# pallgeuer/novic

Hardware: NVIDIA B200
Metric: labels/sec (greedy, batch 4096) (higher is better)
Workload: dtype bf16

## Files before the change

novic_b200/csrc/abi.cu:

```cuda
#include <cstdarg>
#include <cstdio>
#include <cstring>
#include <map>
#include <mutex>
#include <string>
#include <tuple>
#include <vector>

#include "../../include/novic_b200.h"
#include "train.cuh"
#include "optim.cuh"
#include "vit.cuh"
#include "blockrows.cuh"

using namespace novic;

namespace {

thread_local std::string g_err;
int64_t g_launches = 0;

int fail(const char* fmt, ...) {
  char buf[1024];
  va_list ap;
// ... 107 lines not shown

int make_tmap_3d(CUtensorMap* map, const void* base, const cuuint64_t (&dims)[3], const cuuint64_t (&strides)[2], const cuuint32_t (&box)[3]) {
  if (load_driver_entry()) return 1;
  if ((reinterpret_cast<uintptr_t>(base) & 15) != 0 || strides[0] % 16 != 0 || strides[1] % 16 != 0) return fail("TMA operand base / strides must be 16-byte aligned");
  if (box[0] * 2 != 128) return fail("128-byte swizzle needs a 64-element inner box");
  cuuint32_t estr[3] = {1, 1, 1};
  CUresult r = g_encode(map, CU_TENSOR_MAP_DATA_TYPE_BFLOAT16, 3, const_cast<void*>(base), dims, strides, box, estr, CU_TENSOR_MAP_INTERLEAVE_NONE,
                        CU_TENSOR_MAP_SWIZZLE_128B, CU_TENSOR_MAP_L2_PROMOTION_L2_256B, CU_TENSOR_MAP_FLOAT_OOB_FILL_NONE);
  if (r != CUDA_SUCCESS) return fail("cuTensorMapEncodeTiled (3-D) failed with CUresult %d", (int)r);
  return 0;
}

constexpr int kStagesQKV = 5, kStagesGelu = 5, kStagesRow = 4, kStagesLogits = 5;
bool g_fuse_block = true;
int g_block_rows64_min = 148 * 32 + 1;
int g_attn_split_max = 0;
int g_qkv_ws_div = 24;
int g_qkv_ws_stages = 3;
int g_vit_direct = 1;
bool g_attn_prefix = true;
bool g_attn_split = true;
bool g_fuse_attn = false;
bool g_ffn1_ksplit = true;
int g_block64_pad = 16384;
int g_block_rows = 0;
constexpr int kBlock64MaxRows = 1536;
int g_qkv_ws = 1;
bool g_wgrad_mn = true;
int g_qkv_per_tile = 0;
int g_qkv_mc = 0;
int g_qkv_bn = 128;
bool g_fuse_qkv = false;
bool g_attn_tf = true;
int g_attn_hint = 1;
int g_row_stages = 4;
bool g_split_ffn = true;
bool g_early_b = true;
bool g_wide_gemm = true;
constexpr int kWideKbs = 2, kWideStages = 3;
int g_num_sms = 148;
int g_logits_ew = 16;
int g_logits_bn = 256;
int g_grid_div = 1;
constexpr int kLogitBN = kTileN;

bool g_use_pdl = true;
int g_cur_class = 9;
unsigned g_skip_classes = 0;
template <class... KArgs, class... Args>
cudaError_t launch_k(void (*kernel)(KArgs...), dim3 grid, dim3 block, size_t smem, cudaStream_t s, Args&&... args) {
  if ((g_skip_classes >> g_cur_class) & 1u) return cudaSuccess;
  cudaLaunchConfig_t cfg{};
  cfg.gridDim = grid; cfg.blockDim = block; cfg.dynamicSmemBytes = smem; cfg.stream = s;
  cudaLaunchAttribute attr[1];
  attr[0].id = cudaLaunchAttributeProgrammaticStreamSerialization;
  attr[0].val.programmaticStreamSerializationAllowed = 1;
  cfg.attrs = attr; cfg.numAttrs = g_use_pdl ? 1 : 0;
  return cudaLaunchKernelEx(&cfg, kernel, static_cast<KArgs>(args)...);
}

template <class Epi, int STAGES, int KBS = 1, int BN = kTileN, int EW = kEpiWarps>
int set_gemm_attr() {
  static_assert(gemm_persistent_smem_bytes(STAGES, KBS, BN, EW) <= 227 * 1024, "GEMM pipeline does not fit in shared memory");
  CUDA_TRY(cudaFuncSetAttribute(gemm_kernel<Epi, STAGES, KBS, BN, EW>, cudaFuncAttributeMaxDynamicSharedMemorySize, gemm_persistent_smem_bytes(STAGES, KBS, BN, EW)));
  return 0;
}

// ... 283 lines not shown
};

struct Workspace {
  int64_t B = 0, nseq = 0, rows = 0, logit_rows = 0;
  int H = 1, rps = 0, ntiles = 0, hcap = 0, chains = 1;
  float* ein; __nv_bfloat16* ebf; float* x; __nv_bfloat16 *xn, *xfin, *q, *ao, *hb; __nv_bfloat16* kv;
  LogitPartial* part; float* topv; int* topi;
  long long* g_tok; unsigned char *g_pad, *g_done; float *g_score, *g_nll, *g_len, *g_score_out; int* flags;
  long long* b_tok[2]; unsigned char *b_pad[2], *b_anc[2], *b_fin[2]; float *b_score[2], *b_len[2], *b_norm;
  unsigned char *keypad, *effpad, *correct; long long* tgt_masked; float *nll_rows, *loss;
  uint32_t* allow = nullptr; int allow_words = 0; int* allow_edge0 = nullptr; int* g_node = nullptr; int* b_node[2] = {nullptr, nullptr};
  size_t bytes = 0;
};

struct GraphKey {
  int mode; int64_t B; int H; float tau, alpha; void* ws;
  const void* guide = nullptr; int guide_flags = 0;
  const void* bias = nullptr;
  const void* guide_tok = nullptr; const void* guide_node = nullptr; int num_nodes = 0, num_edges = 0;
  bool operator<(const GraphKey& o) const {
    return std::tie(mode, B, H, tau, alpha, ws, guide, guide_flags, bias, guide_tok, guide_node, num_nodes, num_edges) <
           std::tie(o.mode, o.B, o.H, o.tau, o.alpha, o.ws, o.guide, o.guide_flags, o.bias, o.guide_tok, o.guide_node, o.num_nodes, o.num_edges);
  }
};

struct NovicHandle {
  NovicCfg cfg;
  int device = 0;
  bool weights_set = false;
  bool use_graphs = true;
  bool attn_v1 = false;
  int attn_early = 1;
  int attn_cfg = 0;
  bool attn_stream = true;
  bool fuse_ffn = true;
  bool split_sms = true;
  int num_sms = 148;
  int max_chains = 1;
  cudaStream_t chain_streams[8] = {};
  cudaEvent_t fork_ev = nullptr, join_ev[8] = {};
  int attn_smem_budget = 200 * 1024;
  DropCfg drop_in{nullptr, 0u, 1.f}, drop_layer{nullptr, 0u, 1.f};
  uint32_t* d_drop_seed = nullptr;
  uint32_t drop_seed = 0;
  const void* wbuf_seen = nullptr;
  bool train_graphs = true;
  std::map<std::vector<uint64_t>, std::pair<cudaGraphExec_t, cudaGraphExec_t>> train_graph_cache;
  std::map<std::vector<uint64_t>, int64_t> train_graph_nodes;
  WeightPtrs w;
  cudaStream_t capture_stream = nullptr;
  std::map<GraphKey, cudaGraphExec_t> graphs;
  std::map<GraphKey, int64_t> graph_nodes;
  int* h_flags = nullptr;
  int G() const { return cfg.token_length - 1; }
  int S() const { return cfg.prefix_len + cfg.token_length - 1; }
};

namespace {

int plan_workspace(const NovicHandle* h, int64_t B, int H, int rps, char* base, Workspace* ws) {
  const NovicCfg& c = h->cfg;
  const int P = c.prefix_len, G = h->G(), S = h->S();
  Workspace w;
  w.B = B; w.H = H; w.rps = rps;
  w.nseq = B * H;
  const bool tf = rps > 0;
// ... 36 lines not shown
    w.g_score = reinterpret_cast<float*>(P_(4 * B));
    w.g_nll = reinterpret_cast<float*>(P_(4 * B));
    w.g_len = reinterpret_cast<float*>(P_(4 * B));
    w.g_score_out = reinterpret_cast<float*>(P_(4 * B));
  } else if (!tf) {
    for (int i = 0; i < 2; ++i) {
      w.b_tok[i] = reinterpret_cast<long long*>(P_(8 * w.nseq * G));
      w.b_pad[i] = reinterpret_cast<unsigned char*>(P_(w.nseq * G));
      w.b_anc[i] = reinterpret_cast<unsigned char*>(P_(w.nseq * G));
      w.b_fin[i] = reinterpret_cast<unsigned char*>(P_(w.nseq));
      w.b_score[i] = reinterpret_cast<float*>(P_(4 * w.nseq));
      w.b_len[i] = reinterpret_cast<float*>(P_(4 * w.nseq));
    }
    w.b_norm = reinterpret_cast<float*>(P_(4 * w.nseq));
  } else {
    w.keypad = reinterpret_cast<unsigned char*>(P_(w.nseq * S));
    w.effpad = reinterpret_cast<unsigned char*>(P_(w.logit_rows));
    w.correct = reinterpret_cast<unsigned char*>(P_(w.logit_rows));
    w.tgt_masked = reinterpret_cast<long long*>(P_(8 * w.logit_rows));
    w.nll_rows = reinterpret_cast<float*>(P_(4 * w.logit_rows));
    w.loss = reinterpret_cast<float*>(P_(4 * 2));
  }
  w.bytes = b.off;
  *ws = w;
  return 0;
}

struct PassCfg {
  int M;
  int nseq, nq, q0, slot_mul, beams;
  const unsigned char* keypad; int keypad_ld;
  const unsigned char* anc; int anc_ld;
  int remap_in, remap_skip, remap_out;
};

AttnParams attention_params(NovicHandle* h, const Workspace& ws, const PassCfg& pc, int l) {
  const NovicCfg& c = h->cfg;
  const int S = h->S();
  const size_t kv_layer = static_cast<size_t>(ws.nseq) * S * kE;
  __nv_bfloat16* kc = ws.kv + (static_cast<size_t>(l) * 2 + 0) * kv_layer;
  __nv_bfloat16* vc = ws.kv + (static_cast<size_t>(l) * 2 + 1) * kv_layer;
  AttnParams pa{};
  pa.q = ws.q; pa.kcache = kc; pa.vcache = vc; pa.out = ws.ao; pa.keypad = pc.keypad; pa.anc = pc.anc;
  pa.nseq = pc.nseq; pa.nq = pc.nq; pa.q0 = pc.q0; pa.smax = S; pa.P = c.prefix_len; pa.beams = pc.beams;
  pa.prefix_bidir = c.strictly_causal ? 0 : 1; pa.keypad_ld = pc.keypad_ld; pa.anc_ld = pc.anc_ld;
  pa.slot_mul = pc.slot_mul;
  pa.early_loads = h->attn_early;
  pa.scale_log2e = 1.4426950408889634f / sqrtf(static_cast<float>(kHeadDim));
  pa.stream_hint = g_attn_hint;
  return pa;
}

int launch_attention(NovicHandle* h, const Workspace& ws, const PassCfg& pc, int l, cudaStream_t s) {
  const NovicCfg& c = h->cfg;
  const AttnParams pa = attention_params(h, ws, pc, l);
  KSpan t(kKAttn, s);
  const int nkeys_step = (pa.prefix_bidir && pc.q0 < pa.P) ? pa.P : pc.q0 + 1;
  if (h->attn_stream && g_attn_split && pc.nq == 1 && pc.keypad == nullptr && nkeys_step <= kSpMaxKeys &&
      pc.nseq <= (g_attn_split_max > 0 ? g_attn_split_max : 2 * kSpSeqs * std::max(1, h->num_sms / g_grid_div))) {
    CUDA_TRY(launch_k(attention_split_kernel, dim3(static_cast<unsigned>(ceil_div(pc.nseq, kSpSeqs))), dim3(kSpWarps * 32), kSpSmemBytes, s, pa));
  } else if (h->attn_stream && pc.nq == 1 && pc.keypad == nullptr) {
    auto go = [&](auto kernel, int warps, int slots, int chunk) {
      const int grid = static_cast<int>(std::min<int64_t>(std::max(1, h->num_sms / g_grid_div), ceil_div(pc.nseq, warps)));
      return launch_k(kernel, dim3(grid), dim3(warps * 32), as_smem_bytes(warps, slots, chunk), s, pa);
    };
    switch (h->attn_cfg) {
      case 1: CUDA_TRY(go(attention_stream_kernel_t<12, 2, 8>, 12, 2, 8)); break;
      case 2: CUDA_TRY(go(attention_stream_kernel_t<16, 2, 6>, 16, 2, 6)); break;
      case 3: CUDA_TRY(go(attention_stream_kernel_t<8, 3, 8>, 8, 3, 8)); break;
      case 4: CUDA_TRY(go(attention_stream_kernel_t<24, 2, 4>, 24, 2, 4)); break;
      case 5: CUDA_TRY(go(attention_stream_kernel_t<14, 3, 4>, 14, 3, 4)); break;
      case 6: CUDA_TRY(go(attention_stream_kernel_t<14, 4, 4>, 14, 4, 4)); break;
      case 7: CUDA_TRY(go(attention_stream_kernel_t<28, 2, 4>, 28, 2, 4)); break;
      case 8: CUDA_TRY(go(attention_stream_kernel_t<16, 2, 4>, 16, 2, 4)); break;
      default: CUDA_TRY(go(attention_stream_kernel_t<16, 3, 4>, 16, 3, 4)); break;
    }
  } else if (g_attn_prefix && pc.q0 == 0 && pc.nq == c.prefix_len && pc.nq <= kApMaxP && pc.keypad == nullptr && pc.anc == nullptr) {
    const int grid = static_cast<int>(std::min<int64_t>(std::max(1, h->num_sms / g_grid_div), ceil_div(pc.nseq, kApWarps)));
    CUDA_TRY(launch_k(attention_prefix_kernel, dim3(grid), dim3(kApWarps * 32), kApSmemBytes, s, pa));
  } else if (g_attn_tf && pc.q0 == 0 && pc.nq > c.prefix_len && pc.nq <= kAttnBwdMaxS && pc.beams == 1 && pc.slot_mul == 1 && pc.anc == nullptr) {
    const unsigned grid = static_cast<unsigned>(ceil_div(static_cast<int64_t>(pc.nseq) * kHeads, kAttnTfWarps));
    attention_tf_kernel<false><<<grid, kAttnTfWarps * 32, kAttnTfSmemBytes, s>>>(pa);
// ... 5 lines not shown
    const int stage_bytes = nk_max * 2048;
    const int budget = h->attn_smem_budget;
    int nstages = std::max(2, std::min(kAttnMaxStages, (budget - 512) / stage_bytes));
    const int ncons = std::min(kAttnConsumers, nstages);
    nstages = nstages / ncons * ncons;
    const int smem = nstages * stage_bytes + 2 * kAttnMaxStages * 8;
    const int grid = static_cast<int>(std::min<int64_t>(std::max(1, h->num_sms / g_grid_div), ceil_div(pc.nseq, 2)));
    CUDA_TRY(launch_k(attention_bulk_kernel, dim3(grid), dim3(kAttnThreads), smem, s, pa, nstages, stage_bytes, ncons));
  }
  ++g_launches;
  return 0;
}

int run_layers(NovicHandle* h, const Workspace& ws, const PassCfg& pc, cudaStream_t s) {
  const NovicCfg& c = h->cfg;
  const int L = c.num_layers, S = h->S(), M = pc.M;
  CUtensorMap tm_xn, tm_ao, tm_hb;
  if (make_tmap(&tm_xn, ws.xn, M, kE, kBlockM)) return 1;
  if (make_tmap(&tm_ao, ws.ao, M, kE, kBlockM)) return 1;
  if (make_tmap(&tm_hb, ws.hb, M, c.ffn_dim, kBlockM)) return 1;
  CUtensorMap tm_xn3, tm_ao64;
  if (make_tmap3(&tm_xn3, ws.xn, M, kE, kBlockM, kWideKbs)) return 1;
  if (make_tmap3(&tm_ao64, ws.ao, M, kE, kHbRows, 2)) return 1;
  CUtensorMap tm_ao32;
  if (make_tmap3(&tm_ao32, ws.ao, M, kE, kBrRows, kE / kBlockK)) return 1;
  CUtensorMap tm_ao64r;
  if (make_tmap3(&tm_ao64r, ws.ao, M, kE, kB64Rows, kE / kBlockK)) return 1;
  const bool rows64 = g_block_rows64_min > 0 && M >= g_block_rows64_min;
  CUtensorMap tm_x_st;
  if (make_tmap_xblk(&tm_x_st, ws.x, static_cast<int64_t>(ceil_div(M, 32)) * 32)) return 1;
  const size_t kv_layer = static_cast<size_t>(ws.nseq) * S * kE;
  const bool block_fused = g_fuse_block && h->fuse_ffn && c.ffn_dim == kFfnDim;
  const bool qkv_tail = block_fused && g_fuse_qkv && g_wide_gemm;
  auto qkv_params = [&](int l) {
    __nv_bfloat16* kc = ws.kv + (static_cast<size_t>(l) * 2 + 0) * kv_layer;
    __nv_bfloat16* vc = ws.kv + (static_cast<size_t>(l) * 2 + 1) * kv_layer;
    return EpiQKV::Params{ws.q, kc, vc, pc.nq, pc.q0, pc.slot_mul, S, (g_attn_hint & 2) ? 1 : 0};
  };
  for (int l = 0; l < L; ++l) {
    if (l == 0 || !qkv_tail) {
      const EpiQKV::Params pq = qkv_params(l);
      if (g_wide_gemm) {
        KSpan t(kKQkv, s);
        if (g_qkv_ws && kE == kWsKb * kBlockK && ceil_div(M, kBlockM) * g_qkv_ws_div >= 2 * (g_num_sms / g_grid_div / (3 * kE / kTileN))) {
          if (g_qkv_ws == 2) {
            if (launch_gemm_ws2<EpiQKV>(s, tm_xn3, h->w.tm_in_proj3h[l], M, 3 * kE, pq, g_early_b)) return 1;
          } else if (g_qkv_ws_stages == 3) {
            if (launch_gemm_ws<EpiQKV, 3>(s, tm_xn3, h->w.tm_in_proj3[l], M, 3 * kE, pq, g_early_b, &tm_xn)) return 1;
          } else if (launch_gemm_ws<EpiQKV, 2>(s, tm_xn3, h->w.tm_in_proj3[l], M, 3 * kE, pq, g_early_b, &tm_xn)) return 1;
        } else if (g_qkv_bn == 512 && ceil_div(M, kBlockM) * (3 * kE / 256) >= g_num_sms) {
          if (launch_gemm2<EpiQKV, 3>(s, tm_xn3, h->w.tm_in_proj3[l], M, 3 * kE, kE, pq, g_early_b)) return 1;
        } else if (g_qkv_bn == 384 && ceil_div(M, 2 * kBlockM) * (3 * kE / 128) >= g_num_sms / 2) {
          if (launch_gemm2<EpiQKV, 4, 128>(s, tm_xn3, h->w.tm_in_proj3h[l], M, 3 * kE, kE, pq, g_early_b)) return 1;
        } else if (g_qkv_bn == 256 && ceil_div(M, kBlockM) * (3 * kE / 256) >= g_num_sms) {
          if (launch_gemm<EpiQKV, 2, kWideKbs, 256>(s, tm_xn3, h->w.tm_in_proj3w[l], M, 3 * kE, kE, pq, 1, g_early_b)) return 1;
        } else if (launch_gemm<EpiQKV, kWideStages, kWideKbs>(s, tm_xn3, h->w.tm_in_proj3[l], M, 3 * kE, kE, pq, 1, g_early_b)) return 1;
      } else {
        KSpan t(kKQkv, s);
        if (launch_gemm<EpiQKV, kStagesQKV>(s, tm_xn, h->w.tm_in_proj[l], M, 3 * kE, kE, pq, 1, g_early_b)) return 1;
      }
    }
    const bool attn_in_block = block_fused && !qkv_tail && (g_block_rows == 32 || g_block_rows == 0) && g_fuse_attn && h->attn_stream && pc.nq == 1 &&
                               pc.keypad == nullptr;
    if (!attn_in_block && launch_attention(h, ws, pc, l, s)) return 1;
    if (block_fused) {
      FusedBlockParams fb{};
      fb.x = ws.x; fb.gain_mid = h->w.norm2[l]; fb.eps = c.ln_eps;
      if (l + 1 < L) {
        fb.xn = ws.xn; fb.gain_out = h->w.norm1[l + 1];
        if (qkv_tail) { fb.qkv_tail = 1; fb.qkv = qkv_params(l + 1); }
      } else {
        fb.gain_out = h->w.final_norm;
        fb.xn = pc.remap_in > 0 ? ws.xfin : ws.xn;
        fb.remap_rows_in = pc.remap_in; fb.remap_skip = pc.remap_skip; fb.remap_rows_out = pc.remap_out;
      }
      KSpan t(kKFfn2, s);
      if ((g_block_rows == 32 || g_block_rows == 0) && !fb.qkv_tail) {
        const AttnParams pa = attention_params(h, ws, pc, l);
        if (launch_block_rows(s, tm_ao32, h->w.tm_out_proj4[l], h->w.tm_linear1_r3[l], h->w.tm_linear2_4[l], tm_x_st, M, fb, attn_in_block ? &pa : nullptr,
                              (rows64 && !attn_in_block) ? &tm_ao64r : nullptr)) return 1;
        continue;
      }
      if ((g_block_rows == 64 || (g_block_rows <= 0 && M <= kBlock64MaxRows)) && !fb.qkv_tail) {
        if (launch_outproj_ffn64(s, tm_ao64, h->w.tm_out_proj3[l], h->w.tm_linear1_q3[l], h->w.tm_linear2_3[l], M, fb)) return 1;
        continue;
      }
      if (g_ffn1_ksplit && !fb.qkv_tail) {
        if (launch_outproj_ffn_ks(s, tm_ao, h->w.tm_out_proj[l], h->w.tm_linear1[l], h->w.tm_linear2[l], M, fb)) return 1;
        continue;
      }
      if (launch_outproj_ffn(s, tm_ao, h->w.tm_out_proj[l], h->w.tm_linear1_q[l], h->w.tm_linear2[l], h->w.tm_in_proj3[l + 1 < L ? l + 1 : l], M, fb)) return 1;
      continue;
    }
    RowParams po{};
    po.x = ws.x; po.xn = ws.xn; po.gain = h->w.norm2[l]; po.pos = nullptr; po.eps = c.ln_eps;
    { KSpan t(kKOutProj, s); if (launch_rowln(s, tm_ao, h->w.tm_out_proj[l], M, kE, kE, po)) return 1; }
    RowParams pf{};
    pf.x = ws.x; pf.pos = nullptr; pf.eps = c.ln_eps;
    if (l + 1 < L) {
      pf.xn = ws.xn; pf.gain = h->w.norm1[l + 1];
    } else {
      pf.gain = h->w.final_norm;
      pf.xn = pc.remap_in > 0 ? ws.xfin : ws.xn;
      pf.remap_rows_in = pc.remap_in; pf.remap_skip = pc.remap_skip; pf.remap_rows_out = pc.remap_out;
    }
    if (h->fuse_ffn) {
      KSpan t(kKFfn2, s);
// ... 92 lines not shown
  ++g_launches;
  return 0;
}

int enqueue_greedy(NovicHandle* h, const Workspace& ws, float tau, float alpha, float* logits, const GuideCfg& guide, cudaStream_t s) {
  const NovicCfg& c = h->cfg;
  g_grid_div = h->split_sms ? ws.chains : 1;
  const int B = static_cast<int>(ws.B), P = c.prefix_len, G = h->G(), V = c.vocab_size;
  const float inv_tau = 1.0f / tau;
  CUDA_TRY(cudaMemsetAsync(ws.g_done, 0, B, s));
  CUDA_TRY(cudaMemsetAsync(ws.g_score, 0, 4 * B, s));
  CUDA_TRY(cudaMemsetAsync(ws.g_nll, 0, 4 * B, s));
  CUDA_TRY(cudaMemsetAsync(ws.g_len, 0, 4 * B, s));
  CUDA_TRY(cudaMemsetAsync(ws.flags, 1, sizeof(int) * (G + 2), s));
  if (guide.on) CUDA_TRY(cudaMemsetAsync(ws.g_node, 0, sizeof(int) * B, s));
  if (run_prefix(h, ws, 1, P, s)) return 1;
  PassCfg pre{B * P, B, P, 0, 1, 1, nullptr, 0, nullptr, 0, P, P - 1, 1};
  if (run_layers(h, ws, pre, s)) return 1;
  GreedyState st{ws.g_tok, ws.g_pad, ws.g_done, ws.g_score, ws.g_nll, ws.g_len, ws.flags};
  for (int step = 1; step <= G; ++step) {
    const __nv_bfloat16* a = (step == 1) ? ws.xfin : ws.xn;
    float* lg = logits != nullptr ? logits + static_cast<size_t>(step - 1) * V : nullptr;
    if (guide.on && launch_guide_mask(ws, guide, ws.g_node, 1, B, s)) return 1;
    if (run_logits(h, ws, a, B, lg, static_cast<long long>(G) * V, nullptr, inv_tau, (step == 1 && !guide.on) ? 1 : 0, s, &guide)) return 1;
    const float* pos_next = step < G ? h->w.pos + static_cast<size_t>(P + step - 1) * kE : nullptr;
    {
      KSpan t(kKSelect, s);
      CUDA_TRY(launch_k(select_greedy_kernel, dim3(static_cast<unsigned>(ceil_div(B, kSelRows))), dim3(kSelRows * 32), kSelSmemBytes, s,
                        ws.part, ws.ntiles, B, G, step, V, inv_tau, c.label_smoothing, st, h->w.tok_f32, pos_next, h->w.norm1[0], ws.x,
                        ws.xn, c.ln_eps, guide.trie, guide.on ? ws.g_node : static_cast<int*>(nullptr)));
      ++g_launches;
    }
    if (step < G) {
      PassCfg dec{B, B, 1, P + step - 1, 1, 1, nullptr, 0, nullptr, 0, 0, 0, 0};
      if (run_layers(h, ws, dec, s)) return 1;
    }
  }
  CUDA_TRY(launch_k(greedy_finalize_kernel, dim3(static_cast<unsigned>(ceil_div(B, 256))), dim3(256), 0, s, B, alpha, ws.g_score, ws.g_len, ws.g_score_out));
  ++g_launches;
  CUDA_TRY(cudaGetLastError());
  return 0;
}

template <int HCAP>
void launch_select_beam(const Workspace& ws, NovicHandle* h, int step, float inv_tau, float alpha, const BeamState& st,
                        const float* pos_next, const GuideCfg& guide, cudaStream_t s) {
  const NovicCfg& c = h->cfg;
  KSpan t(kKSelect, s);
  launch_k(select_beam_kernel<HCAP>, dim3(static_cast<unsigned>(ceil_div(ws.B, kWarpsPerBlock))), dim3(kWarpsPerBlock * 32), 0, s,
           ws.part, ws.topv, ws.topi, ws.ntiles, static_cast<int>(ws.B), ws.H, h->G(), step, c.vocab_size, inv_tau, alpha, st,
           h->w.tok_f32, pos_next, h->w.norm1[0], ws.x, ws.xn, c.ln_eps, guide.trie);
  ++g_launches;
}

int enqueue_beam(NovicHandle* h, const Workspace& ws, float tau, float alpha, const GuideCfg& guide, cudaStream_t s) {
  const NovicCfg& c = h->cfg;
  g_grid_div = h->split_sms ? ws.chains : 1;
  const int B = static_cast<int>(ws.B), H = ws.H, P = c.prefix_len, G = h->G();
  const int A = B * H;
  const float inv_tau = 1.0f / tau;
  CUDA_TRY(cudaMemsetAsync(ws.flags, 1, sizeof(int) * (G + 2), s));
  beam_init_kernel<<<static_cast<unsigned>(ceil_div(A, 256)), 256, 0, s>>>(B, H, G, ws.b_tok[0], ws.b_pad[0], ws.b_anc[0],
                                                                         ws.b_score[0], ws.b_len[0], ws.b_fin[0], ws.b_node[0]);
  ++g_launches;
  if (run_prefix(h, ws, 1, P, s)) return 1;
  PassCfg pre{B * P, B, P, 0, H, H, nullptr, 0, nullptr, 0, P, P - 1, 1};
  if (run_layers(h, ws, pre, s)) return 1;
// ... 158 lines not shown
    CUDA_TRY(cudaMemcpyToSymbol(g_watchdog_host, &dptr, sizeof(dptr)));
  }
  NovicHandle* h = new NovicHandle();
  h->cfg = *cfg;
  h->device = dev;
  CUDA_TRY(cudaStreamCreateWithFlags(&h->capture_stream, cudaStreamNonBlocking));
  CUDA_TRY(cudaMallocHost(&h->h_flags, sizeof(int) * 8 * (cfg->token_length + 2)));
  CUDA_TRY(cudaMalloc(&h->d_drop_seed, 16));
  CUDA_TRY(cudaMemset(h->d_drop_seed, 0, 16));
  if (const char* e20 = getenv("NOVIC_TRAIN_GRAPHS")) h->train_graphs = e20[0] != '0';
  h->num_sms = prop.multiProcessorCount;
  g_num_sms = prop.multiProcessorCount;
  h->attn_smem_budget = std::min<int>(200 * 1024, static_cast<int>(prop.sharedMemPerBlockOptin) - 8 * 1024);
  CUDA_TRY(cudaFuncSetAttribute(attention_bulk_kernel, cudaFuncAttributeMaxDynamicSharedMemorySize, h->attn_smem_budget + 1024));
  CUDA_TRY(cudaFuncSetAttribute(select_greedy_kernel, cudaFuncAttributeMaxDynamicSharedMemorySize, kSelSmemBytes));
  CUDA_TRY(cudaFuncSetAttribute(attention_stream_kernel_t<16, 3, 4>, cudaFuncAttributeMaxDynamicSharedMemorySize, as_smem_bytes(16, 3, 4)));
  CUDA_TRY(cudaFuncSetAttribute(attention_split_kernel, cudaFuncAttributeMaxDynamicSharedMemorySize, kSpSmemBytes));
  CUDA_TRY(cudaFuncSetAttribute(attention_prefix_kernel, cudaFuncAttributeMaxDynamicSharedMemorySize, kApSmemBytes));
  CUDA_TRY(cudaFuncSetAttribute(attention_stream_kernel_t<12, 2, 8>, cudaFuncAttributeMaxDynamicSharedMemorySize, as_smem_bytes(12, 2, 8)));
  CUDA_TRY(cudaFuncSetAttribute(attention_stream_kernel_t<16, 2, 6>, cudaFuncAttributeMaxDynamicSharedMemorySize, as_smem_bytes(16, 2, 6)));
  CUDA_TRY(cudaFuncSetAttribute(attention_stream_kernel_t<8, 3, 8>, cudaFuncAttributeMaxDynamicSharedMemorySize, as_smem_bytes(8, 3, 8)));
  CUDA_TRY(cudaFuncSetAttribute(attention_stream_kernel_t<24, 2, 4>, cudaFuncAttributeMaxDynamicSharedMemorySize, as_smem_bytes(24, 2, 4)));
  CUDA_TRY(cudaFuncSetAttribute(attention_stream_kernel_t<14, 3, 4>, cudaFuncAttributeMaxDynamicSharedMemorySize, as_smem_bytes(14, 3, 4)));
  CUDA_TRY(cudaFuncSetAttribute(attention_stream_kernel_t<14, 4, 4>, cudaFuncAttributeMaxDynamicSharedMemorySize, as_smem_bytes(14, 4, 4)));
  CUDA_TRY(cudaFuncSetAttribute(attention_stream_kernel_t<28, 2, 4>, cudaFuncAttributeMaxDynamicSharedMemorySize, as_smem_bytes(28, 2, 4)));
  CUDA_TRY(cudaFuncSetAttribute(attention_stream_kernel_t<16, 2, 4>, cudaFuncAttributeMaxDynamicSharedMemorySize, as_smem_bytes(16, 2, 4)));
  if (const char* e12 = getenv("NOVIC_ATTN_CFG")) h->attn_cfg = atoi(e12);
  if (const char* e14 = getenv("NOVIC_WIDE_GEMM")) g_wide_gemm = e14[0] != '0';
  if (const char* e21 = getenv("NOVIC_LOGITS_BN")) g_logits_bn = atoi(e21);
  if (const char* e28 = getenv("NOVIC_LOGITS_EW")) g_logits_ew = atoi(e28);
  if (const char* e15 = getenv("NOVIC_EARLY_B")) g_early_b = e15[0] != '0';
  if (const char* e16 = getenv("NOVIC_SPLIT_FFN")) g_split_ffn = e16[0] != '0';
  if (const char* e17 = getenv("NOVIC_ROW_STAGES")) g_row_stages = atoi(e17);
  if (const char* e18 = getenv("NOVIC_ATTN_HINT")) g_attn_hint = atoi(e18);
  if (const char* e19 = getenv("NOVIC_ATTN_TF")) g_attn_tf = atoi(e19) != 0;
  if (const char* e22 = getenv("NOVIC_FUSE_BLOCK")) g_fuse_block = e22[0] != '0';
  if (const char* e23 = getenv("NOVIC_FUSE_QKV")) g_fuse_qkv = e23[0] != '0';
  if (const char* e24 = getenv("NOVIC_QKV_BN")) g_qkv_bn = atoi(e24);
  if (const char* e27 = getenv("NOVIC_QKV_WS")) g_qkv_ws = atoi(e27);
  if (const char* e27b = getenv("NOVIC_QKV_MC")) g_qkv_mc = atoi(e27b);
  if (const char* e27c = getenv("NOVIC_QKV_PER_TILE")) g_qkv_per_tile = atoi(e27c);
  if (const char* e27d = getenv("NOVIC_WGRAD_MN")) g_wgrad_mn = atoi(e27d) != 0;
  if (const char* e25 = getenv("NOVIC_BLOCK_ROWS")) g_block_rows = atoi(e25);
  if (const char* e25b = getenv("NOVIC_FUSE_ATTN")) g_fuse_attn = e25b[0] != '0';
  if (const char* e25d = getenv("NOVIC_ATTN_SPLIT")) g_attn_split = e25d[0] != '0';
  if (const char* e25h = getenv("NOVIC_ATTN_PREFIX")) g_attn_prefix = e25h[0] != '0';
  if (const char* e25j = getenv("NOVIC_VIT_DIRECT")) g_vit_direct = atoi(e25j) != 0 ? 1 : 0;
  if (const char* e25i = getenv("NOVIC_QKV_WS_DIV")) g_qkv_ws_div = std::max(1, atoi(e25i));
  if (const char* e25g = getenv("NOVIC_QKV_WS_STAGES")) g_qkv_ws_stages = atoi(e25g) == 2 ? 2 : 3;
  if (const char* e25e = getenv("NOVIC_ATTN_SPLIT_MAX")) g_attn_split_max = atoi(e25e);
  if (const char* e25c = getenv("NOVIC_BLOCK_ROWS64_MIN")) g_block_rows64_min = atoi(e25c);
  if (const char* e26 = getenv("NOVIC_BLOCK64_PAD")) g_block64_pad = atoi(e26);
  if (const char* e29 = getenv("NOVIC_FFN1_KSPLIT")) g_ffn1_ksplit = e29[0] != '0';
  if (const char* e13 = getenv("NOVIC_SKIP_CLASSES")) g_skip_classes = static_cast<unsigned>(strtoul(e13, nullptr, 0));
  if (const char* e1 = getenv("NOVIC_ATTN_V1")) h->attn_v1 = e1[0] == '1';
  if (const char* e7 = getenv("NOVIC_ATTN_STREAM")) h->attn_stream = e7[0] != '0';
  if (const char* e9 = getenv("NOVIC_ATTN_EARLY")) h->attn_early = atoi(e9);
  if (const char* e6 = getenv("NOVIC_NO_PDL")) g_use_pdl = e6[0] != '1';
  if (const char* e5 = getenv("NOVIC_NO_SM_SPLIT")) h->split_sms = e5[0] != '1';
  if (const char* e4 = getenv("NOVIC_NO_FFN_FUSION")) h->fuse_ffn = e4[0] != '1';
  if (const char* e3 = getenv("NOVIC_CHAINS")) h->max_chains = std::max(1, std::min(8, atoi(e3)));
  for (int i = 0; i < 8; ++i) {
    CUDA_TRY(cudaStreamCreateWithFlags(&h->chain_streams[i], cudaStreamNonBlocking));
    CUDA_TRY(cudaEventCreateWithFlags(&h->join_ev[i], cudaEventDisableTiming));
  }
  CUDA_TRY(cudaEventCreateWithFlags(&h->fork_ev, cudaEventDisableTiming));
  const char* env = getenv("NOVIC_NO_GRAPHS");
// ... 790 lines not shown
```

novic_b200/csrc/blockrows.cuh:

```cuda
#pragma once

#include "gemm.cuh"
#include "kernels.cuh"

namespace novic {

constexpr int kBrRows = 32;
constexpr int kBrSlotBytes = 64 * 1024;
constexpr int kBrSlots = 3;
constexpr int kBrActBytes = kBrRows * kE * 2;
constexpr int kBrKbBytes = kBrRows * kBlockK * 2;
constexpr int kBrEpiWarps = 16;
constexpr int kBrThreads = 64 + 32 * kBrEpiWarps;
constexpr int kBrRequests = 12;
constexpr int kBrStatsBytes = kBrRows * 4 * 8;
constexpr int kBrBarBytes = 512;
constexpr int kBrAttnSlots = 2;
constexpr int kBrAttnChunk = 4;
__host__ __device__ constexpr int block_rows_smem_bytes() {
  return 1024  + kBrSlots * kBrSlotBytes + kBrActBytes + kBrBarBytes  + kBrStatsBytes;
}
static_assert(block_rows_smem_bytes() <= 227 * 1024, "row-owner block kernel does not fit in shared memory");

__device__ __forceinline__ void tma_load_4d(void* smem_dst, const CUtensorMap* map, uint64_t* bar, int32_t c0, int32_t c1, int32_t c2, int32_t c3,
// ... 237 lines not shown
  const int m0 = blockIdx.x * kBrRows;
  __shared__ int s_trace;
  pdl_trigger();
  if (threadIdx.x == 0) { s_trace = trace_begin() ? 1 : 0; trace_point(s_trace != 0, 0); }

  auto issue = [&](int i) {
    const int slot = (i + kSlotOff) % kBrSlots;
    mbar_arrive_expect_tx(&full_bar[slot], kBrSlotBytes);
    uint8_t* dst = ring + slot * kBrSlotBytes;
    if (i < 8) tma_load_4d(dst, &tmap_wo, &full_bar[slot], 0, 0, i >> 1, (i & 1) * 4, kEvictLast);
    else if (i < 10) tma_load_3d(dst, &tmap_w1, &full_bar[slot], 0, (i - 8) * 4, kEvictLast);
    else tma_load_4d(dst, &tmap_w2, &full_bar[slot], 0, 0, (i - 10) * 2, 0, kEvictLast);
  };

  if (warp == 0) {
    if (elect_one()) {
      if (!ATTN) tma_prefetch_desc(&tmap_ao);
      tma_prefetch_desc(&tmap_wo); tma_prefetch_desc(&tmap_w1); tma_prefetch_desc(&tmap_w2);
      tma_prefetch_desc(&tmap_x);
      for (int st = 0; st < kBrSlots; ++st) { mbar_init(&full_bar[st], 1); mbar_init(&empty_bar[st], 1); }
      mbar_init(act_full, ATTN ? kBrEpiWarps : 1);
      for (int t = 0; t < 4; ++t) { mbar_init(&acc0_full[t], 1); mbar_init(&acc2_full[t], 1); }
      mbar_init(ln2_ready, kBrEpiWarps); mbar_init(acc1_full, 1); mbar_init(h_ready, kBrEpiWarps);
      fence_mbar_init();
      if (ATTN) {
        issue(0);
      } else {
        for (int i = 0; i < kBrSlots; ++i) issue(i);
        pdl_wait();
        mbar_arrive_expect_tx(act_full, kBrActBytes);
        tma_load_3d(act, &tmap_ao, act_full, m0, 0, kEvictFirst);
      }
    }
  } else if (warp == 1) {
    tmem_alloc<512>(tmem_slot);
  }
  tc_fence_before_sync();
  __syncthreads();
  tc_fence_after_sync();
  const uint32_t tmem_base = *tmem_slot;
  long long* const trp = (s_trace != 0 && (threadIdx.x == 64 || threadIdx.x == 32)) ? g_trace : nullptr;
  auto tp = [&](int idx) { if (trp != nullptr) trp[idx] = clock64(); };

  if (warp == 0) {
    if (elect_one()) {
      if (ATTN) {
        mbar_wait(act_full, 0, 1);
        issue(1); issue(2);
      }
      for (int i = kBrSlots; i < kBrRequests; ++i) {
        mbar_wait(&empty_bar[(i + kSlotOff) % kBrSlots], ((i / kBrSlots) - 1) & 1, 1);
        issue(i);
      }
    }
  } else if (warp == 1) {
    if (elect_one()) {
      const uint32_t lb = (smem_u32(act) & 0x3FFFFu) >> 4;
      auto lo = [](const void* p) { return (smem_u32(p) & 0x3FFFFu) >> 4; };
      constexpr uint32_t kKs = (kUmmaK * 2) >> 4, kAo = kABytes >> 4, kBo = kBrKbBytes >> 4;
      mbar_wait(act_full, 0, 2);
      tp(22);
      for (int i = 0; i < 8; ++i) {
        const int slot = (i + kSlotOff) % kBrSlots;
        mbar_wait(&full_bar[slot], (i / kBrSlots) & 1, 3);
        tp(10 + i);
        tc_fence_after_sync();
// ... 43 lines not shown
        tc_fence_after_sync();
        const uint32_t la = lo(ring + slot * kBrSlotBytes);
#pragma unroll
        for (int tt = 0; tt < 2; ++tt) {
          const uint32_t d = tmem_base + kColFfn2 + ((i - 10) * 2 + tt) * kBrRows;
          umma_lo<false>(d, la + tt * kAo, lb, kIdesc);
#pragma unroll
          for (int q = 1; q < 8; ++q) umma_lo<true>(d, la + (q >> 2) * (2 * kAo) + tt * kAo + (q & 3) * kKs, lb + (q >> 2) * kBo + (q & 3) * kKs, kIdesc);
          umma_commit(&acc2_full[(i - 10) * 2 + tt]);
        }
        umma_commit(&empty_bar[slot]);
      }
    }
  } else {
    const int ew = warp - 2;
    const int quad = warp & 3;
    const int rg = ew >> 2;
    const int fi = quad * 32 + lane;
    const int r0 = rg * 8;
    const uint32_t tmem_lane = tmem_base + (static_cast<uint32_t>(quad * 32) << 16) + static_cast<uint32_t>(r0);
    const float* xrow = ep.x + (static_cast<size_t>(blockIdx.x) * (kE / 4) + fi) * (32 * 4) + r0 * 4;
    const float4 g_mid = __ldg(reinterpret_cast<const float4*>(ep.gain_mid) + fi);
    const float4 g_out = __ldg(reinterpret_cast<const float4*>(ep.gain_out) + fi);
    float r[8][4];
    if (ATTN) {
      br_attention_phase(pa, m0, ew, lane, ring, attn_bar, act);
      fence_proxy_async_smem();
      __syncwarp();
      if (lane == 0) mbar_arrive(act_full);
    } else {
      pdl_wait();
    }
    tp(1);
#pragma unroll
    for (int p = 0; p < 4; ++p) {
      float v[8];
      ld_global_v8(xrow + p * 8, v);
#pragma unroll
      for (int c = 0; c < 4; ++c) { r[2 * p][c] = v[c]; r[2 * p + 1][c] = v[4 + c]; }
    }
    float val[16];
    auto add_tiles = [&](uint64_t* bars, uint32_t col0) {
#pragma unroll
      for (int t = 0; t < 4; ++t) {
        mbar_wait(&bars[t], 0, 8);
        if (t == 0) tp(col0 == 0 ? 25 : 26);
        tc_fence_after_sync();
        float v[8];
        tmem_ld_32x8(tmem_lane + col0 + t * kBrRows, v);
#pragma unroll
        for (int j = 0; j < 8; ++j) {
          const float x = r[j][t] + v[j];
          r[j][t] = x;
          val[j] = t == 0 ? x : val[j] + x;
          val[8 + j] = t == 0 ? x * x : fmaf(x, x, val[8 + j]);
        }
      }
    };
    auto row_stats = [&](float (&a)[8], float (&b)[8], bool store_x) {
      const float tot = br_warp_reduce16(val, lane);
      if ((lane & 1) == 0) {
        const int k = lane >> 1;
        reinterpret_cast<float*>(&s_stats[(r0 + (k & 7)) * 4 + quad])[k >> 3] = tot;
      }
      br_epi_sync();
      if (store_x && threadIdx.x == 64) {
// ... 399 lines not shown
```

novic_b200/csrc/gemm.cuh:

```cuda
#pragma once

#include "ptx.cuh"

namespace novic {

constexpr int kE = 512;
constexpr int kBlockM = 128;
constexpr int kBlockK = 64;
constexpr int kUmmaK = 16;
constexpr int kTileN = 128;
constexpr int kABytes = kBlockM * kBlockK * 2;
constexpr int kBBytes = kTileN * kBlockK * 2;
constexpr int kStageBytes = kABytes + kBBytes;
constexpr int kStagePitch = kTileN * 2 + 16;
constexpr int kWarpStageBytes = 32 * kStagePitch;

__host__ __device__ __forceinline__ size_t xblk_off(int row, int col4) {
  return ((static_cast<size_t>(row >> 5) * (kE / 4) + col4) * 32 + (row & 31)) * 4;
}

__host__ __device__ constexpr int gemm_smem_bytes(int stages) { return stages * kStageBytes + 1024  + 256  + 1536 ; }

struct EpiCtx {
  uint32_t tmem_row;
// ... 1055 lines not shown
          if (keep)
            *reinterpret_cast<uint4*>(ep.xn + static_cast<size_t>(nrow) * kE + c0 + chunk * 8) =
                *reinterpret_cast<const uint4*>(stage + rr * kRowStagePitch + chunk * 16);
        }
      }
      __syncwarp();
    }
  }

  if (threadIdx.x == 64) trace_point(tr, 9);
  tc_fence_before_sync();
  __syncwarp();
  cluster_sync_relaxed();
  if (threadIdx.x == 0) trace_point(tr, 10);
  if (warp == 1) tmem_dealloc<kTmemCols>(tmem_base);
}

constexpr int kFbRing = 4;
constexpr int kFbStages = 7;
__host__ __device__ constexpr int outproj_ffn_smem_bytes() {
  return kFbRing * kStageBytes  + (kFfnDim / kRowCluster) * kE * 2  + 2 * kBBytes  + 2 * kABytes  +
         1024  + 256  + 2 * kRowBN * 4 ;
}
static_assert((kFfnDim / kRowCluster) * kE * 2 == kStageBytes && 2 * kBBytes == kStageBytes && 2 * kABytes == kStageBytes, "regions double as pipeline stages");
struct FusedBlockParams {
  float* x;
  __nv_bfloat16* xn;
  const float* gain_mid;
  const float* gain_out;
  int remap_rows_in, remap_skip, remap_rows_out;
  float eps;
  int qkv_tail;
  EpiQKV::Params qkv;
};

__global__ void __cluster_dims__(kRowCluster, 1, 1) __launch_bounds__(kRowThreads, 1)
outproj_ffn_kernel(const __grid_constant__ CUtensorMap tmap_ao, const __grid_constant__ CUtensorMap tmap_wo, const __grid_constant__ CUtensorMap tmap_w1q,
                   const __grid_constant__ CUtensorMap tmap_w2, const __grid_constant__ CUtensorMap tmap_wqkv, int M, FusedBlockParams ep) {
  constexpr int BN = kRowBN;
  constexpr int kHSplit = kFfnDim / kRowCluster;
  constexpr int kW1kb = kHSplit * kBlockK * 2;
  constexpr uint32_t kIdesc = umma_idesc_bf16_f32(kBlockM, BN);
  constexpr uint32_t kIdescH = umma_idesc_bf16_f32(kBlockM, kHSplit);
  constexpr int kNkb = kE / kBlockK;
  extern __shared__ uint8_t smem_raw[];
  uint8_t* smem = reinterpret_cast<uint8_t*>((reinterpret_cast<uintptr_t>(smem_raw) + 1023) & ~uintptr_t(1023));
  uint8_t* ring = smem;
  uint8_t* w1_smem = ring + kFbRing * kStageBytes;
  uint8_t* w2_smem = w1_smem + kNkb * kW1kb;
  uint8_t* h_smem = w2_smem + 2 * kBBytes;
  uint8_t* after = h_smem + 2 * kABytes;
  uint64_t* full_bar = reinterpret_cast<uint64_t*>(after);
  uint64_t* empty_bar = full_bar + kFbStages;
  uint64_t* tmem_full0 = empty_bar + kFbStages;
  uint64_t* w1_full = tmem_full0 + 1;
  uint64_t* w2_full = tmem_full0 + 2;
  uint64_t* tmem_full1 = tmem_full0 + 3;
  uint64_t* tmem_full2 = tmem_full0 + 4;
  uint64_t* affn_full = tmem_full0 + 5;
  uint64_t* hx_full = tmem_full0 + 6;
  uint64_t* hop_ready = tmem_full0 + 7;
  uint64_t* aq_full = tmem_full0 + 8;
  uint64_t* bq_full = tmem_full0 + 9;
  uint64_t* bq_empty = tmem_full0 + 11;
  uint64_t* tmem_full_q = tmem_full0 + 13;
  uint32_t* tmem_slot = reinterpret_cast<uint32_t*>(tmem_full0 + 16);
// ... 1375 lines not shown
```

novic_b200/csrc/ptx.cuh:

```cuda
#pragma once

#include <cstdint>
#include <cuda.h>
#include <cuda_bf16.h>
#include <cuda_runtime.h>

namespace novic {

__device__ __forceinline__ uint32_t smem_u32(const void* p) {
  return static_cast<uint32_t>(__cvta_generic_to_shared(p));
}

__device__ __forceinline__ uint32_t lane_id() { return threadIdx.x & 31u; }

__device__ __forceinline__ bool elect_one() {
  uint32_t pred;
  asm volatile(
      "{\n\t.reg .pred p;\n\t"
      "elect.sync _|p, 0xffffffff;\n\t"
      "selp.u32 %0, 1, 0, p;\n\t}\n"
      : "=r"(pred));
  return pred != 0;
}

// ... 115 lines not shown
}
__device__ __forceinline__ void tma_load_2d_mc(void* smem_dst, const CUtensorMap* map, uint64_t* bar, int32_t c0, int32_t c1, uint16_t cta_mask,
                                               uint64_t cache_hint) {
  asm volatile(
      "cp.async.bulk.tensor.2d.shared::cluster.global.mbarrier::complete_tx::bytes.multicast::cluster.L2::cache_hint"
      " [%0], [%1, {%3, %4}], [%2], %5, %6;\n" ::"r"(smem_u32(smem_dst)),
      "l"(reinterpret_cast<uint64_t>(map)), "r"(smem_u32(bar)), "r"(c0), "r"(c1), "h"(cta_mask), "l"(cache_hint)
      : "memory");
}

__device__ __forceinline__ void tma_load_3d_at(void* smem_dst, const CUtensorMap* map, uint64_t* bar, int32_t c0, int32_t c1, int32_t c2,
                                               uint64_t cache_hint) {
  asm volatile(
      "cp.async.bulk.tensor.3d.shared::cluster.global.mbarrier::complete_tx::bytes.L2::cache_hint"
      " [%0], [%1, {%3, %4, %5}], [%2], %6;\n" ::"r"(smem_u32(smem_dst)),
      "l"(reinterpret_cast<uint64_t>(map)), "r"(smem_u32(bar)), "r"(c0), "r"(c1), "r"(c2), "l"(cache_hint)
      : "memory");
}

__device__ __forceinline__ void bulk_load_1d(void* smem_dst, const void* gsrc, uint32_t bytes, uint64_t* bar) {
  asm volatile(
      "cp.async.bulk.shared::cluster.global.mbarrier::complete_tx::bytes [%0], [%1], %2, [%3];\n" ::"r"(smem_u32(smem_dst)),
      "l"(reinterpret_cast<uint64_t>(gsrc)), "r"(bytes), "r"(smem_u32(bar))
      : "memory");
}

__device__ __forceinline__ void bulk_load_1d_hint(void* smem_dst, const void* gsrc, uint32_t bytes, uint64_t* bar, uint64_t cache_hint) {
  asm volatile(
      "cp.async.bulk.shared::cluster.global.mbarrier::complete_tx::bytes.L2::cache_hint [%0], [%1], %2, [%3], %4;\n" ::"r"(smem_u32(smem_dst)),
      "l"(reinterpret_cast<uint64_t>(gsrc)), "r"(bytes), "r"(smem_u32(bar)), "l"(cache_hint)
      : "memory");
}

__device__ __forceinline__ void st_global_v4_hint(void* gdst, const uint4& v, uint64_t cache_hint) {
  asm volatile("st.global.L2::cache_hint.v4.b32 [%0], {%1, %2, %3, %4}, %5;\n" ::"l"(gdst), "r"(v.x), "r"(v.y), "r"(v.z), "r"(v.w), "l"(cache_hint)
               : "memory");
}

constexpr uint64_t kEvictFirst = 0x12F0000000000000ull;
constexpr uint64_t kEvictNormal = 0x1000000000000000ull;
constexpr uint64_t kEvictLast = 0x14F0000000000000ull;

template <uint32_t kCols>
__device__ __forceinline__ void tmem_alloc(uint32_t* smem_dst) {
  static_assert(kCols >= 32 && kCols <= 512 && (kCols & (kCols - 1)) == 0, "TMEM columns: power of two in [32,512]");
  asm volatile("tcgen05.alloc.cta_group::1.sync.aligned.shared::cta.b32 [%0], %1;\n" ::"r"(smem_u32(smem_dst)),
               "n"(kCols)
               : "memory");
  asm volatile("tcgen05.relinquish_alloc_permit.cta_group::1.sync.aligned;\n" ::: "memory");
}

template <uint32_t kCols>
__device__ __forceinline__ void tmem_dealloc(uint32_t taddr) {
  asm volatile("tcgen05.dealloc.cta_group::1.sync.aligned.b32 %0, %1;\n" ::"r"(taddr), "n"(kCols) : "memory");
}

__device__ __forceinline__ uint64_t umma_desc_sw128_kmajor(uint32_t smem_addr_bytes) {
  uint64_t d = 0;
  d |= static_cast<uint64_t>((smem_addr_bytes & 0x3FFFFu) >> 4);
  d |= static_cast<uint64_t>(1) << 16;
  d |= static_cast<uint64_t>(1024 >> 4) << 32;
  d |= static_cast<uint64_t>(1) << 46;
  d |= static_cast<uint64_t>(2) << 61;
  return d;
}

// ... 203 lines not shown
```

Before: 845,100.

## Prefetch next layer's KV cache into L2 from the fused FFN block kernel

Adds L2 staging of the next layer's (or the next decode step's first layer's) K/V cache rows, issued from inside the fused block kernel while it runs the FFN. Default mode 2 has epilogue threads issue touch loads over each cached row; modes 0 and 1 use bulk L2 prefetch or per-line prefetch instructions. The goal is to hide the attention kernel's DRAM latency on the KV cache, with the staged size capped by a megabyte budget. The cost is extra loads in the block kernel's epilogue path, and the staged data may push weights out of L2.

```diff
diff --git a/novic_b200/csrc/abi.cu b/novic_b200/csrc/abi.cu
--- a/novic_b200/csrc/abi.cu
+++ b/novic_b200/csrc/abi.cu
@@ -163,7 +163,6 @@
 int g_qkv_bn = 128;
 bool g_fuse_qkv = false;
 bool g_attn_tf = true;
-int g_attn_hint = 1;
 int g_row_stages = 4;
 bool g_split_ffn = true;
 bool g_early_b = true;
@@ -513,6 +512,10 @@
   bool attn_v1 = false;
   int attn_early = 1;
   int attn_cfg = 0;
+  int attn_hint = 1;
+  int kv_stage_mb = 16;
+  bool kv_stage_last = false;
+  int kv_stage_mode = 2;
   bool attn_stream = true;
   bool fuse_ffn = true;
   bool split_sms = true;
@@ -615,6 +618,7 @@
   const unsigned char* keypad; int keypad_ld;
   const unsigned char* anc; int anc_ld;
   int remap_in, remap_skip, remap_out;
+  int next_step;
 };
 
 AttnParams attention_params(NovicHandle* h, const Workspace& ws, const PassCfg& pc, int l) {
@@ -630,7 +634,7 @@
   pa.slot_mul = pc.slot_mul;
   pa.early_loads = h->attn_early;
   pa.scale_log2e = 1.4426950408889634f / sqrtf(static_cast<float>(kHeadDim));
-  pa.stream_hint = g_attn_hint;
+  pa.stream_hint = h->attn_hint;
   return pa;
 }
 
@@ -702,10 +706,13 @@
   const size_t kv_layer = static_cast<size_t>(ws.nseq) * S * kE;
   const bool block_fused = g_fuse_block && h->fuse_ffn && c.ffn_dim == kFfnDim;
   const bool qkv_tail = block_fused && g_fuse_qkv && g_wide_gemm;
+  const int stage_cap = (h->kv_stage_mb > 0 && pc.nq == 1 && pc.keypad == nullptr && pc.beams == 1 && pc.slot_mul == 1 && pc.anc == nullptr)
+                            ? static_cast<int>(std::min<int64_t>(S, (static_cast<int64_t>(h->kv_stage_mb) << 20) / (static_cast<int64_t>(pc.nseq) * 2 * kE * 2)))
+                            : 0;
   auto qkv_params = [&](int l) {
     __nv_bfloat16* kc = ws.kv + (static_cast<size_t>(l) * 2 + 0) * kv_layer;
     __nv_bfloat16* vc = ws.kv + (static_cast<size_t>(l) * 2 + 1) * kv_layer;
-    return EpiQKV::Params{ws.q, kc, vc, pc.nq, pc.q0, pc.slot_mul, S, (g_attn_hint & 2) ? 1 : 0};
+    return EpiQKV::Params{ws.q, kc, vc, pc.nq, pc.q0, pc.slot_mul, S, (h->attn_hint & 2) ? 1 : 0};
   };
   for (int l = 0; l < L; ++l) {
     if (l == 0 || !qkv_tail) {
@@ -743,6 +750,13 @@
         fb.gain_out = h->w.final_norm;
         fb.xn = pc.remap_in > 0 ? ws.xfin : ws.xn;
         fb.remap_rows_in = pc.remap_in; fb.remap_skip = pc.remap_skip; fb.remap_rows_out = pc.remap_out;
+      }
+      const int stage_layer = l + 1 < L ? l + 1 : 0;
+      const int stage_rows = std::min(stage_cap, l + 1 < L ? pc.q0 : (pc.next_step ? pc.q0 + 1 : 0));
+      if (stage_rows > 0) {
+        fb.kv_stage_k = ws.kv + (static_cast<size_t>(stage_layer) * 2 + 0) * kv_layer;
+        fb.kv_stage_v = ws.kv + (static_cast<size_t>(stage_layer) * 2 + 1) * kv_layer;
+        fb.kv_stage_smax = S; fb.kv_stage_rows = stage_rows; fb.kv_stage_last = h->kv_stage_last ? 1 : 0; fb.kv_stage_mode = h->kv_stage_mode;
       }
       KSpan t(kKFfn2, s);
       if ((g_block_rows == 32 || g_block_rows == 0) && !fb.qkv_tail) {
@@ -901,7 +915,7 @@
       ++g_launches;
     }
     if (step < G) {
-      PassCfg dec{B, B, 1, P + step - 1, 1, 1, nullptr, 0, nullptr, 0, 0, 0, 0};
+      PassCfg dec{B, B, 1, P + step - 1, 1, 1, nullptr, 0, nullptr, 0, 0, 0, 0, step + 1 < G ? 1 : 0};
       if (run_layers(h, ws, dec, s)) return 1;
     }
   }
@@ -1126,7 +1140,10 @@
   if (const char* e15 = getenv("NOVIC_EARLY_B")) g_early_b = e15[0] != '0';
   if (const char* e16 = getenv("NOVIC_SPLIT_FFN")) g_split_ffn = e16[0] != '0';
   if (const char* e17 = getenv("NOVIC_ROW_STAGES")) g_row_stages = atoi(e17);
-  if (const char* e18 = getenv("NOVIC_ATTN_HINT")) g_attn_hint = atoi(e18);
+  if (const char* e18 = getenv("NOVIC_ATTN_HINT")) h->attn_hint = atoi(e18);
+  if (const char* e18b = getenv("NOVIC_KV_STAGE_MB")) h->kv_stage_mb = std::max(0, atoi(e18b));
+  if (const char* e18c = getenv("NOVIC_KV_STAGE_LAST")) h->kv_stage_last = e18c[0] == '1';
+  if (const char* e18d = getenv("NOVIC_KV_STAGE_MODE")) h->kv_stage_mode = atoi(e18d);
   if (const char* e19 = getenv("NOVIC_ATTN_TF")) g_attn_tf = atoi(e19) != 0;
   if (const char* e22 = getenv("NOVIC_FUSE_BLOCK")) g_fuse_block = e22[0] != '0';
   if (const char* e23 = getenv("NOVIC_FUSE_QKV")) g_fuse_qkv = e23[0] != '0';
diff --git a/novic_b200/csrc/blockrows.cuh b/novic_b200/csrc/blockrows.cuh
--- a/novic_b200/csrc/blockrows.cuh
+++ b/novic_b200/csrc/blockrows.cuh
@@ -293,6 +293,18 @@
         tma_load_3d(act, &tmap_ao, act_full, m0, 0, kEvictFirst);
       }
     }
+    if (ep.kv_stage_rows > 0 && ep.kv_stage_mode == 0 && m0 + lane < M) {
+      pdl_wait();
+      const size_t off = static_cast<size_t>(m0 + lane) * ep.kv_stage_smax * kE;
+      const uint32_t bytes = static_cast<uint32_t>(ep.kv_stage_rows) * (kE * 2);
+      if (ep.kv_stage_last) {
+        bulk_prefetch_l2_hint(ep.kv_stage_k + off, bytes, kEvictLast);
+        bulk_prefetch_l2_hint(ep.kv_stage_v + off, bytes, kEvictLast);
+      } else {
+        bulk_prefetch_l2(ep.kv_stage_k + off, bytes);
+        bulk_prefetch_l2(ep.kv_stage_v + off, bytes);
+      }
+    }
   } else if (warp == 1) {
     tmem_alloc<512>(tmem_slot);
   }
@@ -402,6 +414,18 @@
       pdl_wait();
     }
     tp(1);
+    if (ep.kv_stage_rows > 0 && ep.kv_stage_mode != 0) {
+      const int t = threadIdx.x - 64;
+      if (m0 + (t >> 4) < M) {
+        const __nv_bfloat16* row = ((t >> 3) & 1 ? ep.kv_stage_v : ep.kv_stage_k) + static_cast<size_t>(m0 + (t >> 4)) * ep.kv_stage_smax * kE + (t & 7) * 64;
+        for (int j = 0; j < ep.kv_stage_rows; ++j) {
+          const __nv_bfloat16* p = row + static_cast<size_t>(j) * kE;
+          if (ep.kv_stage_mode == 2) touch_l2_line(p);
+          else if (ep.kv_stage_last) prefetch_l2_line_last(p);
+          else prefetch_l2_line(p);
+        }
+      }
+    }
 #pragma unroll
     for (int p = 0; p < 4; ++p) {
       float v[8];
diff --git a/novic_b200/csrc/gemm.cuh b/novic_b200/csrc/gemm.cuh
--- a/novic_b200/csrc/gemm.cuh
+++ b/novic_b200/csrc/gemm.cuh
@@ -1111,6 +1111,12 @@
   float eps;
   int qkv_tail;
   EpiQKV::Params qkv;
+  const __nv_bfloat16* kv_stage_k;
+  const __nv_bfloat16* kv_stage_v;
+  int kv_stage_smax;
+  int kv_stage_rows;
+  int kv_stage_last;
+  int kv_stage_mode;
 };
 
 __global__ void __cluster_dims__(kRowCluster, 1, 1) __launch_bounds__(kRowThreads, 1)
diff --git a/novic_b200/csrc/ptx.cuh b/novic_b200/csrc/ptx.cuh
--- a/novic_b200/csrc/ptx.cuh
+++ b/novic_b200/csrc/ptx.cuh
@@ -171,6 +171,21 @@
       : "memory");
 }
 
+__device__ __forceinline__ void bulk_prefetch_l2(const void* gsrc, uint32_t bytes) {
+  asm volatile("cp.async.bulk.prefetch.L2.global [%0], %1;\n" ::"l"(reinterpret_cast<uint64_t>(gsrc)), "r"(bytes) : "memory");
+}
+__device__ __forceinline__ void bulk_prefetch_l2_hint(const void* gsrc, uint32_t bytes, uint64_t cache_hint) {
+  asm volatile("cp.async.bulk.prefetch.L2.global.L2::cache_hint [%0], %1, %2;\n" ::"l"(reinterpret_cast<uint64_t>(gsrc)), "r"(bytes), "l"(cache_hint)
+               : "memory");
+}
+
+__device__ __forceinline__ void prefetch_l2_line(const void* p) { asm volatile("prefetch.global.L2 [%0];\n" ::"l"(p)); }
+__device__ __forceinline__ void prefetch_l2_line_last(const void* p) { asm volatile("prefetch.global.L2::evict_last [%0];\n" ::"l"(p)); }
+__device__ __forceinline__ void touch_l2_line(const void* p) {
+  uint32_t v;
+  asm volatile("ld.global.L2::128B.b32 %0, [%1];\n" : "=r"(v) : "l"(p));
+}
+
 __device__ __forceinline__ void st_global_v4_hint(void* gdst, const uint4& v, uint64_t cache_hint) {
   asm volatile("st.global.L2::cache_hint.v4.b32 [%0], {%1, %2, %3, %4}, %5;\n" ::"l"(gdst), "r"(v.x), "r"(v.y), "r"(v.z), "r"(v.w), "l"(cache_hint)
                : "memory");
```

After: 842,400, median of 6. No clear change (-0.3%).
